# nucypher/TFHE.jl

Hardware: AMD Instinct MI355X
Metric: bootstrapped gates/sec (whole node), N=1024 (higher is better)
Workload: dtype int32 torus / f64 transform; 1 GPU; batch of 4096 independent gate_nand() bootstraps per GPU, tfhe_parameters_80 (n=500, N=1024, k=1, l=2, Bg=2^10, ks t=8, base 2^2); inputs=resident in HBM, launch=one process

## Files before the change

### tfhe.jl_amd/csrc/br_core.hpp

```cpp
#pragma once
#include <stdint.h>
#include <string.h>

#if defined(__HIPCC__)
#include <hip/hip_runtime.h>
#define TFHE_HD __host__ __device__ __forceinline__
typedef double2 cplx;
#else
#define TFHE_HD inline
struct cplx { double x, y; };
#endif

namespace tfhe {

constexpr int kWave = 64;
constexpr int kN = 1024;
constexpr int kM = kN / 2;
constexpr int kPts = kM / kWave;
constexpr int kXchElems = 576;

TFHE_HD cplx mk(double re, double im) { cplx c; c.x = re; c.y = im; return c; }
TFHE_HD cplx cadd(cplx a, cplx b) { return mk(a.x + b.x, a.y + b.y); }
TFHE_HD cplx csub(cplx a, cplx b) { return mk(a.x - b.x, a.y - b.y); }
TFHE_HD cplx cmul(cplx a, cplx b) { return mk(a.x * b.x - a.y * b.y, a.x * b.y + a.y * b.x); }
// ... 312 lines not shown
        const uint32_t v = (uint32_t)p[(B & (NBLK - 1)) * 64];
#if defined(__HIP_DEVICE_COMPILE__)
        uint32_t c_s = (uint32_t)offset - sgn;
        asm("" : "+s"(c_s));
        const uint32_t k = c_s - (uint32_t)cur[m];
        uint32_t r;
        asm("v_xad_u32 %0, %1, %2, %3" : "=v"(r) : "v"(v), "s"(sgn), "v"(k));
        temp[m] = (int32_t)(r ^ (uint32_t)xormask);
#else
        const uint32_t k = ((uint32_t)offset - sgn) - (uint32_t)cur[m];
        temp[m] = (int32_t)(((v ^ sgn) + k) ^ (uint32_t)xormask);
#endif
    }
}
template <int NBLK>
TFHE_HD void load_cur(int lane, const int32_t *img, int32_t (&cur)[NBLK])
{
#pragma unroll
    for (int m = 0; m < NBLK; m++) cur[m] = img[kMir + lane + 64 * m];
}
template <int NBLK>
TFHE_HD void store_cur(int lane, const int32_t (&acc)[NBLK], int32_t *img)
{
#pragma unroll
    for (int m = 0; m < NBLK; m++) img[kMir + lane + 64 * m] = acc[m];
    img[lane] = (int32_t)(0u - (uint32_t)acc[NBLK - 1]);
}

TFHE_HD int32_t digit2(int32_t t, int p, int log2_base)
{
#if defined(__HIP_DEVICE_COMPILE__)
    return __builtin_amdgcn_sbfe(t, (unsigned)(32 - p * log2_base), (unsigned)log2_base);
#else
    return (int32_t)((uint32_t)t << ((p - 1) * log2_base)) >> (32 - log2_base);
#endif
}
TFHE_HD void load_digits2(const int32_t (&temp)[16], int p, int log2_base, cplx (&x)[8])
{
#pragma unroll
    for (int r = 0; r < 8; r++) {
        const double lo = (double)digit2(temp[r], p, log2_base);
        const double hi = (double)digit2(temp[r + 8], p, log2_base);
        if (r == 0) x[r] = mk(lo, -hi);
        else x[r] = mk(lo * twc(r) - hi * tws(r), -(lo * tws(r) + hi * twc(r)));
    }
}
template <int R>
TFHE_HD cplx twist_tan(double a, double b)
{
    if (R == 0) return mk(a, -b);
    if (R == 4) return mk(a - b, -(b + a));
    if (R < 4) return mk(fma_(-twt(R), b, a), -fma_(twt(R), a, b));
    return mk(fma_(twt(R), a, -b), -fma_(twt(R), b, a));
}
TFHE_HD void load_digits2t(const int32_t (&temp)[16], int p, int log2_base, cplx (&u)[8])
{
#define TFHE_TW_(R) u[R] = twist_tan<R>((double)digit2(temp[R], p, log2_base), (double)digit2(temp[R + 8], p, log2_base))
    TFHE_TW_(0); TFHE_TW_(1); TFHE_TW_(2); TFHE_TW_(3); TFHE_TW_(4); TFHE_TW_(5); TFHE_TW_(6); TFHE_TW_(7);
#undef TFHE_TW_
}
constexpr double kTwR0 = 0.70710678118654752440;
constexpr double kTwR1 = 0.84775906502257351226;
constexpr double kTwR3 = 1.1795804271032745923;
constexpr double kTwG0 = 0.92387953251128675613;
constexpr double kTwL = 0.98078528040323044913;
constexpr double kTwSL = 0.69351992266107373091;
TFHE_HD cplx axpy(cplx a, double m, cplx b) { return mk(fma_(m, b.x, a.x), fma_(m, b.y, a.y)); }
TFHE_HD void dft8_fwd_tw(cplx (&x)[8])
{
    const cplx a0 = axpy(x[0], kTwR0, x[4]), a1 = axpy(x[1], kTwR1, x[5]), a2 = cadd(x[2], x[6]), a3 = axpy(x[3], kTwR3, x[7]);
    const cplx t0 = axpy(x[0], -kTwR0, x[4]), t1 = axpy(x[1], -kTwR1, x[5]), t2 = csub(x[2], x[6]), t3 = axpy(x[3], -kTwR3, x[7]);
    const cplx b1 = mk(t1.x + t1.y, t1.y - t1.x);
    const cplx b2 = mk(t2.y, -t2.x);
    const cplx b3 = mk(t3.y - t3.x, -(t3.x + t3.y));
    {
        const cplx c0 = axpy(a0, kTwG0, a2), d0 = axpy(a0, -kTwG0, a2), c1 = axpy(a1, kTwR1, a3), e = axpy(a1, -kTwR1, a3);
        const cplx d1 = mk(e.y, -e.x);
        x[0] = axpy(c0, kTwL, c1); x[4] = axpy(c0, -kTwL, c1); x[2] = axpy(d0, kTwL, d1); x[6] = axpy(d0, -kTwL, d1);
    }
    {
        const cplx c0 = axpy(t0, kTwG0, b2), d0 = axpy(t0, -kTwG0, b2), c1 = axpy(b1, kTwR1, b3), e = axpy(b1, -kTwR1, b3);
        const cplx d1 = mk(e.y, -e.x);
        x[1] = axpy(c0, kTwSL, c1); x[5] = axpy(c0, -kTwSL, c1); x[3] = axpy(d0, kTwSL, d1); x[7] = axpy(d0, -kTwSL, d1);
    }
}
TFHE_HD void fwd2_pass_a(cplx (&x)[8], const LaneTw &w)
{
    dft8<false>(x);
#pragma unroll
    for (int q = 0; q < 8; q++) x[q] = cmul(x[q], w.tw1f[q]);
}
TFHE_HD void fwd2_pass_b(cplx (&x)[8], const LaneTw &w)
{
    dft8<false>(x);
#pragma unroll
    for (int q = 1; q < 8; q++) x[q] = cmul(x[q], w.tw2[q]);
}
TFHE_HD void inv2_pass_b(cplx (&x)[8], const LaneTw &w)
{
#pragma unroll
    for (int q = 1; q < 8; q++) x[q] = cmulc(x[q], w.tw2[q]);
    dft8<true>(x);
}
TFHE_HD void inv2_pass_a(cplx (&x)[8], const LaneTw &w)
{
#pragma unroll
    for (int q = 0; q < 8; q++) x[q] = cmulc(x[q], w.tw1f[q]);
    dft8<true>(x);
}
TFHE_HD double frac_dist(double v)
{
    const double r = (v + 6755399441055744.0) - 6755399441055744.0;
    const double d = v - r;
    return d < 0 ? -d : d;
}

template <bool MARGIN = false, bool FUSED = true>
TFHE_HD void untwist_add2(const cplx (&y)[8], int32_t (&acc)[16], double *worst = nullptr)
{
#pragma unroll
    for (int r = 0; r < 8; r++) {
        if (FUSED) {
            double zr, zi;
            if (r == 0) { zr = y[r].x; zi = y[r].y; }
            else if (r == 4) { zr = y[r].x - y[r].y; zi = y[r].y + y[r].x; }
            else if (r < 4) { zr = fma_(-twt(r), y[r].y, y[r].x); zi = fma_(twt(r), y[r].x, y[r].y); }
            else { zr = fma_(twt(r), y[r].x, -y[r].y); zi = fma_(twt(r), y[r].y, y[r].x); }
            if (MARGIN) {
                const double a = frac_dist(zr * twk(r)), b = frac_dist(zi * twk(r));
                if (a > *worst) *worst = a;
                if (b > *worst) *worst = b;
            }
            acc[r] = (int32_t)((uint32_t)acc[r] + (uint32_t)round_scaled_to_torus32(zr, twk(r)));
            acc[r + 8] = (int32_t)((uint32_t)acc[r + 8] + (uint32_t)round_scaled_to_torus32(zi, -twk(r)));
        } else {
            double re, im;
            if (r == 0) { re = y[r].x; im = -y[r].y; }
            else { re = y[r].x * twc(r) - y[r].y * tws(r); im = -(y[r].x * tws(r) + y[r].y * twc(r)); }
            if (MARGIN) {
                const double a = frac_dist(re), b = frac_dist(im);
                if (a > *worst) *worst = a;
                if (b > *worst) *worst = b;
            }
            acc[r] = (int32_t)((uint32_t)acc[r] + (uint32_t)round_to_torus32(re));
            acc[r + 8] = (int32_t)((uint32_t)acc[r + 8] + (uint32_t)round_to_torus32(im));
        }
    }
}

}
```

### tfhe.jl_amd/csrc/engine.hpp

```cpp
#pragma once
#include <hip/hip_runtime.h>

#include <algorithm>
#include <atomic>
#include <cstdarg>
#include <cstdio>
#include <cstring>
#include <new>
#include <string>
#include <thread>
#include <vector>

#include "../../include/tfhe_mi355x.h"
#include "experiment.hpp"
#include "br_core.hpp"

using namespace tfhe;

#include "kernels_blind_rotate.hpp"
#include "kernels_anyn.hpp"
#include "kernels_n512.hpp"
#include "kernels_keyswitch.hpp"

struct ErrBuf {
// ... 149 lines not shown
    int n512_rw = 0;
    int k2_w3 = -1;
    int k2_rw = 0;
    int v3_rw = 0;
    int64_t pipeline_min = 4096;
    bool last_call_two_streams = false;
    struct MapStage { void *h = nullptr; size_t cap = 0; hipEvent_t ev = nullptr; bool pending = false; };
    static constexpr int kMapStages = 4;
    MapStage map_stage[kMapStages];
    unsigned map_next = 0;
    MapStage *map_cur = &map_stage[0];
    void *h_map = nullptr;
    hipEvent_t map_ev = nullptr;

    std::atomic<std::thread::id> owner{};
    int owner_depth = 0;

    bool multi() const { return !kids.empty(); }

    int set_err(int code, const char *fmt, ...)
    {
        ErrBuf next;
        va_list ap;
        va_start(ap, fmt);
        vsnprintf(next.s, sizeof next.s, fmt, ap);
        va_end(ap);
        err = next;
        return code;
    }
};

#define HIP_TRY(ctx, call)                                                                         \
    do {                                                                                           \
        hipError_t e_ = (call);                                                                    \
        if (e_ != hipSuccess)                                                                      \
            return (ctx)->set_err(TFHE_ERR_DEVICE, "%s failed: %s (%s:%d)", #call, hipGetErrorString(e_), __FILE__, __LINE__); \
    } while (0)


extern thread_local const tfhe_ctx *g_rejected_ctx;
extern const char kBusyMessage[];
struct CallGuard {
    tfhe_ctx *c;
    bool ok;
    explicit CallGuard(tfhe_ctx *c_) : c(c_), ok(false)
    {
        const std::thread::id me = std::this_thread::get_id();
        if (c->owner.load(std::memory_order_acquire) == me) { c->owner_depth++; ok = true; return; }
        std::thread::id none{};
        ok = c->owner.compare_exchange_strong(none, me, std::memory_order_acq_rel);
        if (ok) { c->owner_depth = 1; if (g_rejected_ctx == c) g_rejected_ctx = nullptr; }
        else g_rejected_ctx = c;
    }
    ~CallGuard()
    {
        if (ok && --c->owner_depth == 0) c->owner.store(std::thread::id{}, std::memory_order_release);
    }
    CallGuard(const CallGuard &) = delete;
    CallGuard &operator=(const CallGuard &) = delete;
};
#define ENTER_CTX(ctx)                                                                             \
    if (!(ctx)) return TFHE_ERR_INVALID_ARG;                                                       \
    alloc_checkpoint();                                                                            \
    CallGuard call_guard_(ctx);                                                                    \
    if (!call_guard_.ok) return TFHE_ERR_STATE

int32_t abi_caught(tfhe_ctx *c, const char *who) noexcept;
#define ABI_CATCH(ctx, who) catch (...) { return abi_caught(ctx, who); }
extern std::atomic<int64_t> g_fail_alloc_countdown;
inline void alloc_checkpoint()
{
    if (g_fail_alloc_countdown.load(std::memory_order_relaxed) > 0 && g_fail_alloc_countdown.fetch_sub(1, std::memory_order_relaxed) == 1) throw std::bad_alloc();
}

int32_t ensure_dyn_lds(tfhe_ctx *c, const void *fn, size_t bytes, const char *what);
#define LDS_TRY(ctx, bytes, ...)                                                                   \
    do {                                                                                           \
        const int32_t rl_ = ensure_dyn_lds(ctx, (const void *)(__VA_ARGS__), (size_t)(bytes), #__VA_ARGS__); \
        if (rl_) return rl_;                                                                       \
    } while (0)

constexpr size_t kH2TableOffset = kTableElems + 1024;
constexpr size_t kN512TableOffset = kH2TableOffset + kH2TableElems;

inline int ilog2i(int x) { int r = 0; while ((1 << r) < x) r++; return r; }
inline bool op_has_a(int op) { return !(op == TFHE_GATE_CONST0 || op == TFHE_GATE_CONST1); }
inline bool op_has_b(int op) { return op_has_a(op) && !(op == TFHE_GATE_NOT || op == TFHE_GATE_COPY); }
inline size_t bk_poly_count(const tfhe_params &p) { return (size_t)p.n * p.bs_l * (p.k + 1) * (p.k + 1); }

template <typename F>
struct ScopeExit {
    F f;
    ~ScopeExit() { f(); }
};
template <typename F>
ScopeExit<F> on_exit(F f) { return ScopeExit<F>{f}; }

template <typename F>
static int32_t fan_out(tfhe_ctx *c, const std::vector<int> &which, F &&fn)
{
    std::vector<int32_t> rcs(which.size(), TFHE_OK);
    std::vector<std::thread> th;
    std::vector<size_t> inline_ones;
    th.reserve(which.size());
    inline_ones.reserve(which.size());
    auto shard = [&](size_t i) noexcept {
        try { rcs[i] = fn(which[i]); } catch (...) { rcs[i] = abi_caught(c->kids[(size_t)which[i]], "fan-out shard"); }
    };
    for (size_t i = 1; i < which.size(); i++) {
        try {
            th.emplace_back([&shard, i] { shard(i); });
        } catch (...) {
            inline_ones.push_back(i);
        }
    }
    if (!which.empty()) shard(0);
    for (size_t i : inline_ones) shard(i);
    for (auto &t : th) t.join();
    std::fill(c->kid_ran.begin(), c->kid_ran.end(), 0);
    for (int k : which) c->kid_ran[(size_t)k] = 1;
    for (size_t i = 0; i < which.size(); i++)
        if (rcs[i]) return c->set_err(rcs[i], "device %d (kid %d): %s", c->kids[(size_t)which[i]]->device, which[i], c->kids[(size_t)which[i]]->err.c_str());
    return TFHE_OK;
}
inline std::vector<int> all_kids(const tfhe_ctx *c)
{
    std::vector<int> v(c->kids.size());
    for (size_t i = 0; i < v.size(); i++) v[i] = (int)i;
    return v;
}

template <typename F>
static int32_t multi_rows(tfhe_ctx *c, int64_t B, F &&call)
{
    const int nk = (int)c->kids.size();
    std::vector<int> which;
    std::vector<int64_t> lo((size_t)nk), hi((size_t)nk);
    for (int r = 0; r < nk; r++) {
        lo[(size_t)r] = B * r / nk; hi[(size_t)r] = B * (r + 1) / nk;
        if (hi[(size_t)r] > lo[(size_t)r]) which.push_back(r);
    }
    return fan_out(c, which, [&](int r) { return call(c->kids[(size_t)r], lo[(size_t)r], hi[(size_t)r] - lo[(size_t)r]); });
}

void shard_bounds_by_rotations(const uint8_t *opcodes, int64_t B, int shards, int64_t *bounds);
void quiesce(tfhe_ctx *c);
int32_t tgsw_prepare(tfhe_ctx *c, const int32_t *d_polys, cplx *d_out, size_t npolys, hipStream_t s);
void mk_tgsw_drop(tfhe_ctx *c);
struct DiagArgs;
int32_t prepare_diag(tfhe_ctx *c, size_t R, hipStream_t s, DiagArgs &d);
void name_kernel(tfhe_ctx *c, const char *fmt, ...) __attribute__((format(printf, 2, 3)));
struct TvPtrs { const int32_t *tv; const int32_t *index; int32_t *bodies = nullptr; int32_t n_out = 1; };
template <class A>
static WithTv<A> with_tv(const A &a, const TvPtrs &tv)
{
    WithTv<A> t;
    static_cast<A &>(t) = a;
    t.tv = tv.tv;
    t.tv_index = tv.index;
    t.bodies = tv.bodies;
    t.n_out = tv.n_out;
    return t;
}
int32_t launch_blind_rotate(tfhe_ctx *c, size_t R, int32_t mu, hipStream_t s, const TvPtrs *tv = nullptr);
int32_t launch_keyswitch(tfhe_ctx *c, size_t G, const int32_t *e0, const int32_t *e1, const int32_t *dst, const int32_t *ext, int32_t *out, hipStream_t s);
int32_t enter_stream(tfhe_ctx *c, hipStream_t s);
// ... 45 lines not shown
```

### tfhe.jl_amd/csrc/engine_context.hip

```cpp
#include "engine.hpp"
#include <cmath>

thread_local ErrBuf g_create_error;
thread_local const tfhe_ctx *g_rejected_ctx = nullptr;
static thread_local const tfhe_ctx *g_caught_ctx = nullptr;
static thread_local ErrBuf g_caught_error;
std::atomic<int64_t> g_fail_alloc_countdown{0};
const char kBusyMessage[] = "the context is inside another call on another thread: calls on one context must not overlap (one caller at a time; use one context per thread)";

int32_t abi_caught(tfhe_ctx *c, const char *who) noexcept
{
    int32_t code = TFHE_ERR_STATE;
    ErrBuf &e = c ? g_caught_error : g_create_error;
    try {
        throw;
    } catch (const std::bad_alloc &) {
        code = TFHE_ERR_NOMEM;
        e.format("%s: out of host memory (std::bad_alloc); nothing was changed that a repeated call would not redo", who);
    } catch (const std::exception &x) {
        e.format("%s: unexpected C++ exception: %s", who, x.what());
    } catch (...) {
        e.format("%s: unexpected C++ exception", who);
    }
    g_caught_ctx = c;
    if (c) {
        const tfhe_ctx *rejected = g_rejected_ctx;
        CallGuard again(c);
        if (again.ok) c->err = g_caught_error;
        g_rejected_ctx = rejected;
    }
    return code;
}

static void build_tables(std::vector<cplx> &h)
{
    h.resize(kN512TableOffset + kN512TableElems);
    fill_tables<long double>(h.data(), [](long double a) { return cosl(a); }, [](long double a) { return sinl(a); });
    const long double pi = 3.14159265358979323846264338327950288L;
    for (int w = 0; w < 2; w++)
        for (int q = 0; q < 8; q++)
            for (int t = 0; t < 64; t++) {
                const long double a = -pi * (long double)(t * (1 + 4 * w + 8 * q)) / 2048.0L;
                h[kTableElems + w * 512 + q * 64 + t] = mk((double)cosl(a), (double)sinl(a));
            }
    auto put = [&](size_t idx, long double turns_of_pi) { const long double a = -pi * turns_of_pi; h[idx] = mk((double)cosl(a), (double)sinl(a)); };
    for (int hh = 0; hh < 2; hh++)
        for (int q = 0; q < 4; q++)
            for (int t = 0; t < 64; t++)
                put(kH2TableOffset + (size_t)(hh * 4 + q) * 64 + t, (long double)t / 1024.0L + (hh ? (long double)t / 256.0L : 0.0L) + (long double)(t * q) / 128.0L);
    for (int q = 0; q < 4; q++)
        for (int t = 0; t < 16; t++) put(kH2TableOffset + 512 + (size_t)q * 16 + t, (long double)(t * q) / 32.0L);
    for (int q = 0; q < 4; q++)
        for (int t = 0; t < 4; t++) put(kH2TableOffset + 576 + (size_t)q * 4 + t, (long double)(t * q) / 8.0L);
    for (int q = 0; q < 4; q++)
        for (int t = 0; t < 64; t++) put(kN512TableOffset + (size_t)q * 64 + t, (long double)t / 512.0L + (long double)(t * q) / 128.0L);
}

void shard_bounds_by_rotations(const uint8_t *opcodes, int64_t B, int shards, int64_t *bounds)
{
    auto cost = [&](int64_t g) -> int64_t {
        const int op = opcodes ? opcodes[g] : TFHE_GATE_NAND;
        const int rot = op == TFHE_GATE_MUX ? 2 : (op == TFHE_GATE_NOT || op == TFHE_GATE_COPY || op == TFHE_GATE_CONST0 || op == TFHE_GATE_CONST1) ? 0 : 1;
        return 1000 * (int64_t)rot + 1;
    };
    int64_t total = 0;
    for (int64_t g = 0; g < B; g++) total += cost(g);
    bounds[0] = 0;
    int64_t cum = 0, g = 0;
    for (int r = 1; r < shards; r++) {
        while (g < B && cum * shards < total * r) { cum += cost(g); g++; }
        bounds[r] = g;
    }
    bounds[shards] = B;
}

extern "C" {

int32_t tfhe_abi_version(void) { return TFHE_ABI_VERSION_REPORTED; }

int32_t tfhe_device_count(void)
{
    int n = 0;
    if (hipGetDeviceCount(&n) != hipSuccess) return -1;
    return n;
}

const char *tfhe_last_error(const tfhe_ctx *ctx)
{
    if (!ctx) return g_create_error.c_str();
    if (g_rejected_ctx == ctx) return kBusyMessage;
    if (g_caught_ctx == ctx) return g_caught_error.c_str();
    return ctx->err.c_str();
}

int32_t tfhe_shard_bounds(const uint8_t *opcodes, int64_t B, int32_t shards, int64_t *bounds) try
{
    alloc_checkpoint();
    if (B < 0 || shards < 1 || !bounds) return TFHE_ERR_INVALID_ARG;
    shard_bounds_by_rotations(opcodes, B, shards, bounds);
    return TFHE_OK;
}
ABI_CATCH(nullptr, "tfhe_shard_bounds")

static void exactness_class(const tfhe_params &p, int &cls, double &bound_log2, double &margin)
{
    const double np = (double)(p.parties > 1 ? p.parties + 1 : p.k + 1) * p.bs_l, N = (double)p.N, beta = (double)p.bs_log2_base;
    bound_log2 = std::log2(np * N) + (beta - 1.0) + 31.0;
    const double rms = std::sqrt(np * N) * std::exp2(beta + 32.0) / 12.0;
    margin = 4.5 * std::exp2(-53.0) * rms * std::max(4.0, std::log2(N / 2.0));
    const bool margin_ok = margin < 0.25, typical_ok = 8.0 * rms < std::exp2(51.0);
    cls = !(margin_ok && typical_ok) ? 0 : bound_log2 < 51.0 ? 2 : 1;
}

int32_t tfhe_ctx_create(const tfhe_params *params, int32_t device_id, tfhe_ctx **out_ctx) try
{
    alloc_checkpoint();
    if (!params || !out_ctx) { g_create_error = "tfhe_ctx_create: NULL argument"; return TFHE_ERR_INVALID_ARG; }
    *out_ctx = nullptr;
    const tfhe_params &p = *params;
    char buf[256];
// ... 217 lines not shown
```

### tfhe.jl_amd/csrc/engine_dispatch.hip

```cpp
#define TFHE_EMIT_KEYSWITCH_KERNELS
#include "engine.hpp"
#include "br_launch.hpp"

#include <map>
#include <mutex>
#include <functional>

int32_t ensure_dyn_lds(tfhe_ctx *c, const void *fn, size_t bytes, const char *what)
{
    static std::mutex mu;
    static std::map<std::pair<int, const void *>, size_t> have;
    std::lock_guard<std::mutex> lk(mu);
    size_t &cur = have[std::make_pair(c->device, fn)];
    if (cur >= bytes) return TFHE_OK;
    const hipError_t e = hipFuncSetAttribute(fn, hipFuncAttributeMaxDynamicSharedMemorySize, (int)bytes);
    if (e != hipSuccess) return c->set_err(TFHE_ERR_DEVICE, "hipFuncSetAttribute(%s, %zu bytes of LDS) failed: %s", what, bytes, hipGetErrorString(e));
    cur = bytes;
    return TFHE_OK;
}

int32_t prepare_diag(tfhe_ctx *c, size_t R, hipStream_t s, DiagArgs &d)
{
    d.margin_bits = nullptr; d.clk = nullptr; d.phase = nullptr;
    c->diag_rows = 0;
    if (!c->measure_margin) return TFHE_OK;
    HIP_TRY(c, c->diag.reserve(R * 24 + 64 * 8));
    HIP_TRY(c, hipMemsetAsync(c->diag.p, 0, R * 24 + 64 * 8, s));
    d.margin_bits = (unsigned long long *)c->diag.p;
    d.clk = d.margin_bits + R;
    d.phase = d.clk + 2 * R;
    c->diag_rows = R;
    return TFHE_OK;
}

void name_kernel(tfhe_ctx *c, const char *fmt, ...)
{
    char buf[128];
    va_list ap;
    va_start(ap, fmt);
    vsnprintf(buf, sizeof buf, fmt, ap);
    va_end(ap);
    c->last_kernel = buf;
}

static int br_inst_l(const tfhe_ctx *c)
{
    return (c->P.bs_l == 2 || c->P.bs_l == 3) && !c->br_rt_l ? c->P.bs_l : 0;
}

static void name_br(tfhe_ctx *c, const char *family, int L, const char *rest = "")
{
    if (L) name_kernel(c, "blind_rotate_kernel_%s<%d%s>", family, L, rest);
    else name_kernel(c, "blind_rotate_kernel_%s<0%s>(l=%d)", family, rest, c->P.bs_l);
}

static int32_t launch_blind_rotate_part(tfhe_ctx *c, size_t first, size_t R, int32_t mu, hipStream_t s, const DiagArgs &diag, int k2_kind = -1 ,
                                        const TvPtrs *tv_all = nullptr)
{
    TvPtrs tv{nullptr, nullptr};
    if (tv_all) tv = TvPtrs{tv_all->tv, tv_all->index + first, tv_all->bodies ? tv_all->bodies + first * (size_t)tv_all->n_out : nullptr, tv_all->n_out};
    BrArgs a;
    a.diag = diag;
    if (diag.margin_bits) { a.diag.margin_bits += first; a.diag.clk += 2 * first; }
    const bool dg = c->measure_margin;
    a.bara = (const int32_t *)c->bara.p + first * (size_t)(c->P.n + 1);
    a.bk = c->d_bk;
    a.ext = (int32_t *)c->ext.p + first * ((size_t)c->P.k * c->P.N + 1);
    a.T = c->T;
    a.g = c->g;
    a.n = c->P.n;
    a.mu = mu;
    a.prio_steps = (int32_t)((int64_t)c->P.n * c->br_prio_pct / 100);
    a.R = (int32_t)R;
    const int L = c->P.bs_l;
    a.l = L;
    if (c->anyn()) {
        const int K1 = c->P.k + 1, N = c->P.N, M = N / 2;
        anyn::Args g;
        g.diag = a.diag; g.bara = a.bara; g.bk = a.bk; g.ext = a.ext; g.g = c->g; g.n = a.n; g.mu = mu; g.K1 = K1; g.L = L; g.R = (int32_t)R;
        g.log2N = ilog2i(N); g.parties = 1;
        g.wtab = c->d_anyn_tab; g.twist = c->d_anyn_tab + M;
        HIP_TRY(c, c->mk_acc.reserve((first + R) * (size_t)K1 * N * sizeof(int32_t)));
        g.acc = (int32_t *)c->mk_acc.p + first * (size_t)K1 * N;
        const bool fits = anyn::lds_bytes(N, K1) <= 160 * 1024;
        const bool spec_lds = c->anyn_spec < 0 ? fits : (c->anyn_spec == 0 && fits);
        g.spec_g = nullptr;
        if (!spec_lds) {
            HIP_TRY(c, c->spec.reserve((first + R) * (size_t)K1 * (M > 0 ? M : 1) * sizeof(cplx)));
            g.spec_g = (cplx *)c->spec.p + first * (size_t)K1 * (M > 0 ? M : 1);
        }
        const BrLaunch geo{0, 1, dg, dim3((unsigned)R), dim3((unsigned)anyn::threads_for(N)), anyn::lds_bytes(N, spec_lds ? K1 : 0)};
        const int32_t rc = tv_all ? br_launch_anyn(c, with_tv(g, tv), geo, s) : br_launch_anyn(c, g, geo, s);
        if (rc) return rc;
        name_kernel(c, spec_lds ? "blind_rotate_kernel_anyn(N=%d,k=%d,l=%d)" : "blind_rotate_kernel_anyn(N=%d,k=%d,l=%d,spec=global)", N, c->P.k, L);
        return TFHE_OK;
    }
    if (c->n512()) {
        N512Args b;
        b.diag = a.diag; b.bara = a.bara; b.bk = a.bk; b.ext = a.ext; b.g = c->g; b.n = a.n; b.mu = mu; b.R = (int32_t)R; b.l = L;
        b.prio_steps = a.prio_steps;
        b.tw1 = c->d_tables + kN512TableOffset; b.tw2q = c->d_tables + kH2TableOffset + 512; b.tw3q = b.tw2q + 64;
        if (c->n512_w2 == 1 || (c->n512_w2 < 0 && R <= 6 * (size_t)c->cu_count)) {
            const BrLaunch geo{br_inst_l(c), 1, dg, dim3((unsigned)R), dim3(128), kN512W2LdsBytes};
            const int32_t rc = tv_all ? br_launch_n512w2(c, with_tv(b, tv), geo, s) : br_launch_n512w2(c, b, geo, s);
            if (rc) return rc;
            name_br(c, "n512w2", geo.L);
            return TFHE_OK;
        }
        const bool group = !dg && (c->n512_rw == 4 || (c->n512_rw == 0 && R >= 8 * (size_t)c->cu_count));
        const int rw = group ? 4 : 1;
        const BrLaunch geo{br_inst_l(c), rw, dg, dim3((unsigned)((R + rw - 1) / rw)), dim3(64 * rw), (size_t)rw * kN512LdsBytes};
        const int32_t rc = tv_all ? br_launch_n512(c, with_tv(b, tv), geo, s) : br_launch_n512(c, b, geo, s);
        if (rc) return rc;
        name_br(c, "n512", geo.L, group ? ",rw4" : "");
        return TFHE_OK;
    }
    const bool tuned = c->P.N == kN2 ? (c->P.k == 1 && L == 3) : c->P.k == 1 ? true : (c->P.k == 2 && (L == 2 || L == 3));
    if (!tuned || c->br_general) {
        const int K1 = c->P.k + 1, H = c->P.N / kN;
        const size_t img = (size_t)kMir + c->P.N;
        BrGenArgs g;
        g.diag = a.diag; g.bara = a.bara; g.bk = a.bk; g.ext = a.ext; g.g = c->g; g.n = a.n; g.mu = mu; g.K1 = K1; g.L = L; g.R = (int32_t)R;
        HIP_TRY(c, c->mk_acc.reserve((first + R) * K1 * img * sizeof(int32_t)));
        g.acc = (int32_t *)c->mk_acc.p + first * K1 * img;
        g.tw1f = c->P.N == kN2 ? (const cplx *)(c->d_tables + kTableElems) : c->T.tw1f;
        g.tw2 = c->T.tw2;
        const BrLaunch geo{0, 1, dg, dim3((unsigned)R), dim3(64), (kXchElems + 64 + (size_t)K1 * H * kM) * sizeof(cplx)};
        const bool n2048 = c->P.N == kN2;
        const int32_t rc = tv_all ? br_launch_general(c, with_tv(g, tv), n2048, geo, s) : br_launch_general(c, g, n2048, geo, s);
        if (rc) return rc;
        name_kernel(c, "blind_rotate_kernel_general(N=%d,k=%d,l=%d)", c->P.N, c->P.k, L);
        return TFHE_OK;
    }
    if (c->P.N == kN2) {
        Br2048Args b;
        b.diag = a.diag; b.bara = a.bara; b.bk = a.bk; b.ext = a.ext; b.tw1f2 = c->d_tables + kTableElems; b.tw2 = c->T.tw2; b.g = c->g; b.n = a.n; b.mu = mu; b.prio_steps = a.prio_steps;
        b.R = (int32_t)R;
        const int rw = dg ? 1 : c->n2048_rw ? c->n2048_rw : (R <= (size_t)c->cu_count ? 1 : 2);
        const size_t ldsb = (size_t)rw * (2 * kImg2 * 4 + 2 * kXchElems * sizeof(cplx)) + 64 * sizeof(cplx) + 64;
        const BrLaunch geo{L, rw, dg, dim3((unsigned)((R + rw - 1) / rw)), dim3(128 * rw), ldsb};
        const int32_t rc = tv_all ? br_launch_n2048x(c, with_tv(b, tv), geo, s) : br_launch_n2048x(c, b, geo, s);
        if (rc) return rc;
        name_br(c, "n2048x", L, rw == 2 ? ",rw2" : ",rw1");
        return TFHE_OK;
    }
    if (c->P.k == 2) {
        const size_t cus = (size_t)c->cu_count;
        const bool w3 = k2_kind >= 0 ? k2_kind == 1 : (c->k2_w3 == 1 || (c->k2_w3 < 0 && R <= 2 * cus));
        if (w3) {
            const BrLaunch geo{L, 1, dg, dim3((unsigned)R), dim3(192), kK2W3LdsBytes};
            const int32_t rc = tv_all ? br_launch_k2w3(c, with_tv(a, tv), geo, s) : br_launch_k2w3(c, a, geo, s);
// ... 177 lines not shown
```

### tfhe.jl_amd/csrc/kernels_common.hpp

```cpp
#pragma once

#include <hip/hip_runtime.h>

#include "../../include/tfhe_mi355x.h"
#include <type_traits>

#include "br_core.hpp"

using namespace tfhe;

template <class A>
struct WithTv : A {
    const int32_t *tv;
    const int32_t *tv_index;
    int32_t *bodies;
    int32_t n_out;
};
#ifdef TFHE_TV_KERNELS
#define TV_KERNEL(name) name##_tv
#define TV_ARGS(A) WithTv<A>
constexpr bool kTV = true;
#else
#define TV_KERNEL(name) name
#define TV_ARGS(A) A
constexpr bool kTV = false;
#endif
template <class A>
__device__ __forceinline__ const int32_t *tv_of(const A &, size_t, int) { return nullptr; }
template <class A>
__device__ __forceinline__ const int32_t *tv_of(const WithTv<A> &P, size_t w, int N)
{
    return P.tv + (size_t)__builtin_amdgcn_readfirstlane(P.tv_index[w]) * N;
}
template <class A>
__device__ __forceinline__ void store_bodies(const A &, size_t, int, const int32_t *, int) {}
template <class A>
__device__ __forceinline__ void store_bodies(const WithTv<A> &P, size_t w, int lane, const int32_t *body, int N)
{
    if (P.bodies && lane < P.n_out) P.bodies[w * P.n_out + lane] = body[lane * (N / P.n_out)];
}

struct DiagArgs {
    unsigned long long *margin_bits;
    unsigned long long *clk;
    unsigned long long *phase;
};

#ifdef TFHE_STAMP
#define STAMP_DECL unsigned long long st_prev_ = __builtin_amdgcn_s_memtime(), st_acc_[16] = {0, 0, 0, 0, 0, 0, 0, 0, 0, 0, 0, 0, 0, 0, 0, 0}
#define STAMP(k) do { if (MARGIN) { const unsigned long long t_ = __builtin_amdgcn_s_memtime(); st_acc_[k] += t_ - st_prev_; st_prev_ = t_; } } while (0)
#define STAMP_FLUSH(diag, wave) do { if (MARGIN && blockIdx.x == 0 && (threadIdx.x & 63) == 0 && (diag).phase) { for (int k_ = 0; k_ < 16; k_++) (diag).phase[(wave) * 16 + k_] = st_acc_[k_]; } } while (0)
#else
#define STAMP_DECL do { } while (0)
#define STAMP(k) do { } while (0)
#define STAMP_FLUSH(diag, wave) do { } while (0)
#endif

template <bool DIAG>
__device__ __forceinline__ void diag_begin(unsigned long long &t0, unsigned long long &r0)
{
    if constexpr (DIAG) {
        t0 = __builtin_amdgcn_s_memtime();
        r0 = __builtin_amdgcn_s_memrealtime();
    }
}
template <bool DIAG>
__device__ __forceinline__ void diag_end(const DiagArgs &d, size_t w, double worst, unsigned long long t0, unsigned long long r0, bool clock_writer = (threadIdx.x == 0))
{
    if constexpr (DIAG) {
#pragma unroll
        for (int off = 32; off > 0; off >>= 1) {
            const double o = __shfl_xor(worst, off);
            worst = o > worst ? o : worst;
        }
        if ((threadIdx.x & 63) == 0) {
            atomicMax(&d.margin_bits[w], (unsigned long long)__double_as_longlong(worst));
            if (clock_writer) {
                d.clk[2 * w] = __builtin_amdgcn_s_memtime() - t0;
                d.clk[2 * w + 1] = __builtin_amdgcn_s_memrealtime() - r0;
            }
        }
    }
}

__device__ __forceinline__ int wave_in_block() { return __builtin_amdgcn_readfirstlane((int)(threadIdx.x >> 6)); }
__device__ __forceinline__ int32_t load_uniform_i32(const int32_t *p)
{
    return *(const __attribute__((address_space(4))) int32_t *)(p);
}

__device__ __forceinline__ int lane_id() { return (int)__builtin_amdgcn_mbcnt_hi(~0u, __builtin_amdgcn_mbcnt_lo(~0u, 0u)); }
__device__ __forceinline__ int lane_id_fresh()
{
    unsigned z = 0;
    asm volatile("" : "+s"(z));
    return (int)__builtin_amdgcn_mbcnt_hi(~0u, __builtin_amdgcn_mbcnt_lo(~0u, z));
}

template <int I, int N, typename F>
__device__ __forceinline__ void static_for(F &&f)
{
    if constexpr (I < N) {
        f(std::integral_constant<int, I>{});
        static_for<I + 1, N>(f);
    }
}

__device__ __forceinline__ double opaque_scalar(double v) { asm("" : "+s"(v)); return v; }
struct Tan16 { double t[5], r0, r1, r3, g0, l, sl, c[5]; };
template <bool WITH_COS = false>
__device__ __forceinline__ Tan16 load_tan16()
{
    Tan16 k;
    k.t[0] = 0.0; k.t[4] = 1.0; k.c[0] = 1.0;
    if (WITH_COS) { k.c[1] = opaque_scalar(twk(1)); k.c[2] = opaque_scalar(twk(2)); k.c[3] = opaque_scalar(twk(3)); k.c[4] = opaque_scalar(twk(4)); }
    k.t[1] = opaque_scalar(twt(1)); k.t[2] = opaque_scalar(twt(2)); k.t[3] = opaque_scalar(twt(3));
    k.r0 = opaque_scalar(kTwR0); k.r1 = opaque_scalar(kTwR1); k.r3 = opaque_scalar(kTwR3);
    k.g0 = opaque_scalar(kTwG0); k.l = opaque_scalar(kTwL); k.sl = opaque_scalar(kTwSL);
    return k;
}
template <int R>
__device__ __forceinline__ cplx twist_tan_o(double a, double b, const Tan16 &k)
{
    if (R == 0) return mk(a, -b);
    if (R == 4) return mk(a - b, -(b + a));
    const double t = k.t[R < 4 ? R : 8 - R];
    if (R < 4) return mk(fma_(-t, b, a), -fma_(t, a, b));
    return mk(fma_(t, a, -b), -fma_(t, b, a));
}
__device__ __forceinline__ void load_digits2t_o(const int32_t (&temp)[16], int p, int log2_base, cplx (&u)[8], const Tan16 &k)
{
    static_for<0, 8>([&](auto rc) {
        constexpr int R = decltype(rc)::value;
        u[R] = twist_tan_o<R>((double)digit2(temp[R], p, log2_base), (double)digit2(temp[R + 8], p, log2_base), k);
    });
}
__device__ __forceinline__ void dft8_fwd_tw_o(cplx (&x)[8], const Tan16 &k)
{
    const cplx a0 = axpy(x[0], k.r0, x[4]), a1 = axpy(x[1], k.r1, x[5]), a2 = cadd(x[2], x[6]), a3 = axpy(x[3], k.r3, x[7]);
    const cplx t0 = axpy(x[0], -k.r0, x[4]), t1 = axpy(x[1], -k.r1, x[5]), t2 = csub(x[2], x[6]), t3 = axpy(x[3], -k.r3, x[7]);
    const cplx b1 = mk(t1.x + t1.y, t1.y - t1.x);
    const cplx b2 = mk(t2.y, -t2.x);
    const cplx b3 = mk(t3.y - t3.x, -(t3.x + t3.y));
    {
        const cplx c0 = axpy(a0, k.g0, a2), d0 = axpy(a0, -k.g0, a2), c1 = axpy(a1, k.r1, a3), e = axpy(a1, -k.r1, a3);
        const cplx d1 = mk(e.y, -e.x);
        x[0] = axpy(c0, k.l, c1); x[4] = axpy(c0, -k.l, c1); x[2] = axpy(d0, k.l, d1); x[6] = axpy(d0, -k.l, d1);
    }
    {
        const cplx c0 = axpy(t0, k.g0, b2), d0 = axpy(t0, -k.g0, b2), c1 = axpy(b1, k.r1, b3), e = axpy(b1, -k.r1, b3);
        const cplx d1 = mk(e.y, -e.x);
        x[1] = axpy(c0, k.sl, c1); x[5] = axpy(c0, -k.sl, c1); x[3] = axpy(d0, k.sl, d1); x[7] = axpy(d0, -k.sl, d1);
    }
}

template <bool MARGIN>
__device__ __forceinline__ void untwist_add2_o(const cplx (&y)[8], int32_t (&acc)[16], double *worst, const Tan16 &k)
{
    static_for<0, 8>([&](auto rc) {
        constexpr int r = decltype(rc)::value;
        const double t = k.t[r < 4 ? r : 8 - r], c = k.c[r < 4 ? r : 8 - r];
        double zr, zi;
        if (r == 0) { zr = y[r].x; zi = y[r].y; }
        else if (r == 4) { zr = y[r].x - y[r].y; zi = y[r].y + y[r].x; }
        else if (r < 4) { zr = fma_(-t, y[r].y, y[r].x); zi = fma_(t, y[r].x, y[r].y); }
        else { zr = fma_(t, y[r].x, -y[r].y); zi = fma_(t, y[r].y, y[r].x); }
        if (MARGIN) {
            const double a = frac_dist(zr * c), b = frac_dist(zi * c);
            if (a > *worst) *worst = a;
            if (b > *worst) *worst = b;
        }
        if (r == 0) {
            acc[r] = (int32_t)((uint32_t)acc[r] + (uint32_t)round_to_torus32(zr));
            acc[r + 8] = (int32_t)((uint32_t)acc[r + 8] + (uint32_t)round_to_torus32(-zi));
        } else {
            acc[r] = (int32_t)((uint32_t)acc[r] + (uint32_t)round_scaled_to_torus32(zr, c));
            acc[r + 8] = (int32_t)((uint32_t)acc[r + 8] + (uint32_t)round_scaled_to_torus32(zi, -c));
        }
    });
}

struct BrArgs {
    DiagArgs diag;
    const int32_t *bara;
    const cplx *bk;
    int32_t *ext;
    Tables T;
    Gadget g;
    int32_t n;
    int32_t mu;
    int32_t prio_steps;
    int32_t R;
    int32_t l;
    int32_t grp_big, grp_q;
};

__device__ __forceinline__ void wave_priority_begin(int prio_steps)
{
    if (prio_steps > 0) __builtin_amdgcn_s_setprio(3);
}
__device__ __forceinline__ void wave_priority_step(int step, int prio_steps)
{
    if (prio_steps <= 0) return;
    if (step == prio_steps / 3) __builtin_amdgcn_s_setprio(2);
    else if (step == 2 * prio_steps / 3) __builtin_amdgcn_s_setprio(1);
    else if (step == prio_steps) __builtin_amdgcn_s_setprio(0);
}

#define WAVE_LDS_FENCE() asm volatile("" ::: "memory")

constexpr int kImg = kMir + kN;

template <int NBLK>
__device__ __forceinline__ void rotate_poly(int lane, int a, const int32_t *img, int32_t offset, int32_t xormask, int32_t (&temp)[NBLK])
{
    int32_t cur[NBLK];
    load_cur<NBLK>(lane, img, cur);
    int a_here = __builtin_amdgcn_readfirstlane(a);
    asm volatile("" : "+s"(a_here));
    rotate_sub3<NBLK>(lane, a_here, img, cur, offset, xormask, temp);
}
template <bool MARGIN, bool FUSED = true>
__device__ __forceinline__ void accumulate_poly(int lane, const cplx (&y)[8], int32_t *img, double *worst)
{
    int32_t accr[16];
    load_cur<16>(lane, img, accr);
    untwist_add2<MARGIN, FUSED>(y, accr, worst);
    store_cur<16>(lane, accr, img);
}
__device__ __forceinline__ void init_body_poly(int lane, int barb, int32_t mu, int32_t *img)
{
    int32_t b[16];
#pragma unroll
    for (int m = 0; m < 16; m++) {
        const int idx = (lane + 64 * m + barb) & (2 * kN - 1);
        b[m] = (idx & kN) ? (int32_t)(0u - (uint32_t)mu) : mu;
    }
    store_cur<16>(lane, b, img);
}
__device__ __forceinline__ int32_t tv_coef(const int32_t *v, int idx, int N)
{
    const int32_t x = v[idx & (N - 1)];
    return (idx & N) ? (int32_t)(0u - (uint32_t)x) : x;
}
template <class A>
__device__ __forceinline__ void init_body(int lane, int barb, const A &P, size_t w, int32_t *img)
{
    if constexpr (kTV) {
        const int32_t *v = tv_of(P, w, kN);
        int32_t b[16];
#pragma unroll
        for (int m = 0; m < 16; m++) b[m] = tv_coef(v, (lane + 64 * m + barb) & (2 * kN - 1), kN);
        store_cur<16>(lane, b, img);
    } else {
        init_body_poly(lane, barb, P.mu, img);
    }
}
__device__ __forceinline__ void init_zero_poly(int lane, int32_t *img)
{
    int32_t z[16];
#pragma unroll
    for (int m = 0; m < 16; m++) z[m] = 0;
    store_cur<16>(lane, z, img);
}
__device__ __forceinline__ void extract_mask_poly(int lane, const int32_t *img, int32_t *ext)
{
#pragma unroll
    for (int m = 0; m < 16; m++) {
        const int j = lane + 64 * m;
        const int32_t v = img[kMir + j];
// ... 95 lines not shown
```

### tfhe.jl_amd/csrc/kernels_v3.hpp

```cpp
#pragma once
#include "kernels_common.hpp"

constexpr int kV3SyncEvery = 4;
constexpr int kV3LdsBytes = 2 * kImg * 4 + (kXchElems + 64) * (int)sizeof(cplx);

template <int L, int KPF , bool TW2REG = false ,
          bool MARGIN = false , int RW = 1 >
__global__ __launch_bounds__(64 * RW, 2) void TV_KERNEL(blind_rotate_kernel_v3)(TV_ARGS(BrArgs) P)
{
    constexpr int K1 = 2;
    constexpr int KMID = (KPF == 8) ? 4 : 0;
    const int Lr = L ? L : P.l;
    const int F = K1 * Lr;
    wave_priority_begin(P.prio_steps);
    unsigned long long dg_t0 = 0, dg_r0 = 0;
    diag_begin<MARGIN>(dg_t0, dg_r0);
    extern __shared__ __attribute__((aligned(16))) char smem_all[];
        const int wib = (RW > 1) ? wave_in_block() : 0;
    char *smem = smem_all + (size_t)wib * kV3LdsBytes;
    int32_t *acc_lds = reinterpret_cast<int32_t *>(smem);
    cplx *xch = reinterpret_cast<cplx *>(smem + K1 * kImg * 4);
    cplx *tw2_lds = xch + kXchElems;
    const int lane = (RW > 1) ? lane_id() : (int)threadIdx.x;
    size_t w = (size_t)blockIdx.x * RW + wib;
    const bool padding = (RW > 1) && w >= (size_t)P.R;
    if (padding) w = P.R - 1;
    const int32_t *bara = P.bara + w * (P.n + 1);
    const int beta = P.g.log2_base;
    const int32_t xormask = gadget_xor_mask(Lr, beta);

    cplx tw1f[8];
#pragma unroll
    for (int q = 0; q < 8; q++) tw1f[q] = P.T.tw1f[q * 64 + lane];
    tw2_lds[lane] = P.T.tw2[lane];
    cplx tw2r[8];
    if (TW2REG) {
#pragma unroll
        for (int q = 1; q < 8; q++) tw2r[q] = P.T.tw2[q * 8 + (lane & 7)];
    }
    init_zero_poly(lane, acc_lds);
    init_body(lane, bara[P.n] & (2 * kN - 1), P, w, acc_lds + kImg);
    WAVE_LDS_FENCE();

    double worst = 0.0;
    cplx kbuf[16];
    auto key_ptr = [&](int step, int f) {
        const int c = L ? f / (L ? L : 1) : (f >= Lr), p = L ? f % (L ? L : 1) : f - c * Lr;
        return P.bk + (size_t)step * (Lr * K1 * K1 * kM) + (size_t)(p * K1 + c) * K1 * kM + lane;
    };
    {
        const cplx *kp = key_ptr(0, 0);
#pragma unroll
        for (int j = 0; j < KPF; j++) kbuf[j] = kp[j * 64];
    }

    int a_next = bara[0] & (2 * kN - 1);
    for (int i = 0; i < P.n; i++) {
        const int a = a_next;
        a_next = bara[i + 1] & (2 * kN - 1);
        wave_priority_step(i, P.prio_steps);
        if (RW > 1 && (i % kV3SyncEvery) == 0) __builtin_amdgcn_s_barrier();

        cplx out[K1][8];
        int32_t temp[16];
#pragma unroll 1
        for (int f = 0; f < F; f++) {
            const int c = L ? f / (L ? L : 1) : (f >= Lr), p = L ? f % (L ? L : 1) : f - c * Lr;
            if (p == 0) rotate_poly<16>(lane, a, acc_lds + c * kImg, P.g.offset, xormask, temp);
            cplx x[8];
            load_digits2t(temp, p + 1, beta, x);
            dft8_fwd_tw(x);
#pragma unroll
            for (int q = 0; q < 8; q++) x[q] = cmul(x[q], tw1f[q]);
            x1_store_a(lane, x, xch);
            WAVE_LDS_FENCE();
            x1_load_b(lane, x, xch);
            {
                cplx t2[8];
#pragma unroll
                for (int q = 1; q < 8; q++) t2[q] = TW2REG ? tw2r[q] : tw2_lds[q * 8 + (lane & 7)];
                dft8<false>(x);
#pragma unroll
                for (int q = 1; q < 8; q++) x[q] = cmul(x[q], t2[q]);
            }
            WAVE_LDS_FENCE();
            x2_store(lane, x, xch);
            WAVE_LDS_FENCE();
            cplx k1v[8];
            if (KPF == 8 && KMID > 0) {
                const cplx *kp = key_ptr(i, f);
#pragma unroll
                for (int k2 = 0; k2 < KMID; k2++) k1v[k2] = kp[(8 + k2) * 64];
                WAVE_LDS_FENCE();
            }
            x2_load(lane, x, xch);
            WAVE_LDS_FENCE();
            dft8<false>(x);
            if (KPF == 16) {
                if (f == 0) {
#pragma unroll
                    for (int co = 0; co < K1; co++)
#pragma unroll
                        for (int k2 = 0; k2 < 8; k2++) out[co][k2] = cmul(x[k2], kbuf[co * 8 + k2]);
                } else {
#pragma unroll
                    for (int co = 0; co < K1; co++)
#pragma unroll
                        for (int k2 = 0; k2 < 8; k2++) out[co][k2] = cfma(x[k2], kbuf[co * 8 + k2], out[co][k2]);
                }
            } else {
                const cplx *kp = key_ptr(i, f);
#pragma unroll
                for (int k2 = KMID; k2 < 8; k2++) k1v[k2] = kp[(8 + k2) * 64];
                if (f == 0) {
#pragma unroll
                    for (int k2 = 0; k2 < 8; k2++) out[0][k2] = cmul(x[k2], kbuf[k2]);
#pragma unroll
                    for (int k2 = 0; k2 < 8; k2++) out[1][k2] = cmul(x[k2], k1v[k2]);
                } else {
#pragma unroll
                    for (int k2 = 0; k2 < 8; k2++) out[0][k2] = cfma(x[k2], kbuf[k2], out[0][k2]);
#pragma unroll
                    for (int k2 = 0; k2 < 8; k2++) out[1][k2] = cfma(x[k2], k1v[k2], out[1][k2]);
                }
            }
            {
                const bool last = (f + 1 == F);
                const cplx *kp = last ? key_ptr(i + 1 < P.n ? i + 1 : i, 0) : key_ptr(i, f + 1);
#pragma unroll
                for (int j = 0; j < KPF; j++) kbuf[j] = kp[j * 64];
            }
        }
#pragma unroll
        for (int co = 0; co < K1; co++) {
            dft8<true>(out[co]);
            x2_store(lane, out[co], xch);
            WAVE_LDS_FENCE();
            x2_load(lane, out[co], xch);
            {
                cplx t2[8];
#pragma unroll
                for (int q = 1; q < 8; q++) t2[q] = TW2REG ? tw2r[q] : tw2_lds[q * 8 + (lane & 7)];
#pragma unroll
                for (int q = 1; q < 8; q++) out[co][q] = cmulc(out[co][q], t2[q]);
            }
            dft8<true>(out[co]);
            WAVE_LDS_FENCE();
            x1_store_b(lane, out[co], xch);
            WAVE_LDS_FENCE();
            x1_load_a(lane, out[co], xch);
            WAVE_LDS_FENCE();
#pragma unroll
            for (int q = 0; q < 8; q++) out[co][q] = cmulc(out[co][q], tw1f[q]);
            dft8<true>(out[co]);
            accumulate_poly<MARGIN>(lane, out[co], acc_lds + co * kImg, &worst);
        }
        WAVE_LDS_FENCE();
    }

    if (padding) return;
    int32_t *ext = P.ext + w * (kN + 1);
    extract_mask_poly(lane, acc_lds, ext);
    if (lane == 0) ext[kN] = acc_lds[kImg + kMir];
    store_bodies(P, w, lane, acc_lds + kImg + kMir, kN);
    diag_end<MARGIN>(P.diag, w, worst, dg_t0, dg_r0);
}
```

Before: 366,500 gates/s.

## Fold radix-8 twiddles into tangent-scaled DFT8 for middle FFT pass

Replaces the separate second-stage twiddle complex multiply plus plain DFT8 with a per-lane tangent-based scaling (one FMA pair per point) followed by a DFT8 whose butterflies absorb the cosine ratios. This applies in both the forward and inverse middle passes and removes the twiddle LDS reads and cmuls. It also moves the margin tracking into LDS to free registers. The cost is a new precomputed table and possible precision changes from the tangent/ratio factorisation.

Measured after the change: 371,900 gates/s (median of 6 runs). +1.5%, better.

```diff
diff --git a/tfhe.jl_amd/csrc/br_core.hpp b/tfhe.jl_amd/csrc/br_core.hpp
--- a/tfhe.jl_amd/csrc/br_core.hpp
+++ b/tfhe.jl_amd/csrc/br_core.hpp
@@ -418,6 +418,80 @@
         const cplx c0 = axpy(t0, kTwG0, b2), d0 = axpy(t0, -kTwG0, b2), c1 = axpy(b1, kTwR1, b3), e = axpy(b1, -kTwR1, b3);
         const cplx d1 = mk(e.y, -e.x);
         x[1] = axpy(c0, kTwSL, c1); x[5] = axpy(c0, -kTwSL, c1); x[3] = axpy(d0, kTwSL, d1); x[7] = axpy(d0, -kTwSL, d1);
+    }
+}
+constexpr int kTan2Doubles = 16;
+constexpr int kTan2Elems = 8 * kTan2Doubles / 2;
+struct LaneTan2 {
+    double t[6];
+    double r1, r2, r3;
+    double g0, g1, l, sl;
+    cplx w4;
+};
+template <typename LD, typename COS, typename SIN>
+inline void fill_tan2(double *h, COS cosfn, SIN sinfn)
+{
+    const LD pi = (LD)3.14159265358979323846264338327950288L;
+    for (int s = 0; s < 8; s++) {
+        LD c[8], t[8];
+        for (int v = 0; v < 8; v++) {
+            const LD a = (LD)2 * pi * (LD)(v * s) / (LD)64;
+            c[v] = cosfn(a); t[v] = sinfn(a) / cosfn(a);
+        }
+        double *o = h + s * kTan2Doubles;
+        const LD a4 = (LD)-2 * pi * (LD)(4 * s) / (LD)64;
+        o[14] = (double)cosfn(a4); o[15] = (double)sinfn(a4);
+        c[0] = 1; c[4] = 1;
+        o[0] = (double)t[1]; o[1] = (double)t[2]; o[2] = (double)t[3]; o[3] = (double)t[5]; o[4] = (double)t[6]; o[5] = (double)t[7];
+        for (int v = 0; v < 4; v++) o[6 + v] = (double)(c[v + 4] / c[v]);
+        o[10] = (double)(c[2] / c[0]); o[11] = (double)(c[3] / c[1]);
+        o[12] = (double)(c[1] / c[0]); o[13] = (double)(c[1] / c[0] * (LD)0.70710678118654752440084436210484904L);
+    }
+}
+TFHE_HD void load_lane_tan2(int lane, const double *tab, LaneTan2 &k)
+{
+    const double *o = tab + (lane & 7) * kTan2Doubles;
+#pragma unroll
+    for (int j = 0; j < 6; j++) k.t[j] = o[j];
+    k.r1 = o[7]; k.r2 = o[8]; k.r3 = o[9]; k.g0 = o[10]; k.g1 = o[11]; k.l = o[12]; k.sl = o[13];
+    k.w4 = mk(o[14], o[15]);
+}
+template <bool INV>
+TFHE_HD cplx tan2_point(cplx x, double t)
+{
+    return INV ? mk(fma_(-t, x.y, x.x), fma_(t, x.x, x.y)) : mk(fma_(t, x.y, x.x), fma_(-t, x.x, x.y));
+}
+template <bool INV>
+TFHE_HD void tan2_apply(cplx (&x)[8], const LaneTan2 &k)
+{
+    x[1] = tan2_point<INV>(x[1], k.t[0]); x[2] = tan2_point<INV>(x[2], k.t[1]); x[3] = tan2_point<INV>(x[3], k.t[2]);
+    x[4] = INV ? cmulc(x[4], k.w4) : cmul(x[4], k.w4);
+    x[5] = tan2_point<INV>(x[5], k.t[3]); x[6] = tan2_point<INV>(x[6], k.t[4]); x[7] = tan2_point<INV>(x[7], k.t[5]);
+}
+template <bool INV>
+TFHE_HD void dft8_scaled(cplx (&x)[8], const LaneTan2 &k)
+{
+    const cplx a0 = cadd(x[0], x[4]), a1 = axpy(x[1], k.r1, x[5]), a2 = axpy(x[2], k.r2, x[6]), a3 = axpy(x[3], k.r3, x[7]);
+    const cplx t0 = csub(x[0], x[4]), t1 = axpy(x[1], -k.r1, x[5]), t2 = axpy(x[2], -k.r2, x[6]), t3 = axpy(x[3], -k.r3, x[7]);
+    cplx b1, b2, b3;
+    if (!INV) {
+        b1 = mk(t1.x + t1.y, t1.y - t1.x);
+        b2 = mk(t2.y, -t2.x);
+        b3 = mk(t3.y - t3.x, -(t3.x + t3.y));
+    } else {
+        b1 = mk(t1.x - t1.y, t1.x + t1.y);
+        b2 = mk(-t2.y, t2.x);
+        b3 = mk(-(t3.x + t3.y), t3.x - t3.y);
+    }
+    {
+        const cplx c0 = axpy(a0, k.g0, a2), d0 = axpy(a0, -k.g0, a2), c1 = axpy(a1, k.g1, a3), e = axpy(a1, -k.g1, a3);
+        const cplx d1 = INV ? mk(-e.y, e.x) : mk(e.y, -e.x);
+        x[0] = axpy(c0, k.l, c1); x[4] = axpy(c0, -k.l, c1); x[2] = axpy(d0, k.l, d1); x[6] = axpy(d0, -k.l, d1);
+    }
+    {
+        const cplx c0 = axpy(t0, k.g0, b2), d0 = axpy(t0, -k.g0, b2), c1 = axpy(b1, k.g1, b3), e = axpy(b1, -k.g1, b3);
+        const cplx d1 = INV ? mk(-e.y, e.x) : mk(e.y, -e.x);
+        x[1] = axpy(c0, k.sl, c1); x[5] = axpy(c0, -k.sl, c1); x[3] = axpy(d0, k.sl, d1); x[7] = axpy(d0, -k.sl, d1);
     }
 }
 TFHE_HD void fwd2_pass_a(cplx (&x)[8], const LaneTw &w)
diff --git a/tfhe.jl_amd/csrc/engine.hpp b/tfhe.jl_amd/csrc/engine.hpp
--- a/tfhe.jl_amd/csrc/engine.hpp
+++ b/tfhe.jl_amd/csrc/engine.hpp
@@ -255,6 +255,7 @@
 
 constexpr size_t kH2TableOffset = kTableElems + 1024;
 constexpr size_t kN512TableOffset = kH2TableOffset + kH2TableElems;
+constexpr size_t kTan2TableOffset = kN512TableOffset + kN512TableElems;
 
 inline int ilog2i(int x) { int r = 0; while ((1 << r) < x) r++; return r; }
 inline bool op_has_a(int op) { return !(op == TFHE_GATE_CONST0 || op == TFHE_GATE_CONST1); }
diff --git a/tfhe.jl_amd/csrc/engine_context.hip b/tfhe.jl_amd/csrc/engine_context.hip
--- a/tfhe.jl_amd/csrc/engine_context.hip
+++ b/tfhe.jl_amd/csrc/engine_context.hip
@@ -34,8 +34,9 @@
 
 static void build_tables(std::vector<cplx> &h)
 {
-    h.resize(kN512TableOffset + kN512TableElems);
+    h.resize(kTan2TableOffset + kTan2Elems);
     fill_tables<long double>(h.data(), [](long double a) { return cosl(a); }, [](long double a) { return sinl(a); });
+    fill_tan2<long double>(reinterpret_cast<double *>(h.data() + kTan2TableOffset), [](long double a) { return cosl(a); }, [](long double a) { return sinl(a); });
     const long double pi = 3.14159265358979323846264338327950288L;
     for (int w = 0; w < 2; w++)
         for (int q = 0; q < 8; q++)
diff --git a/tfhe.jl_amd/csrc/engine_dispatch.hip b/tfhe.jl_amd/csrc/engine_dispatch.hip
--- a/tfhe.jl_amd/csrc/engine_dispatch.hip
+++ b/tfhe.jl_amd/csrc/engine_dispatch.hip
@@ -67,6 +67,7 @@
     a.bk = c->d_bk;
     a.ext = (int32_t *)c->ext.p + first * ((size_t)c->P.k * c->P.N + 1);
     a.T = c->T;
+    a.tan2 = reinterpret_cast<const double *>(c->d_tables + kTan2TableOffset);
     a.g = c->g;
     a.n = c->P.n;
     a.mu = mu;
diff --git a/tfhe.jl_amd/csrc/kernels_common.hpp b/tfhe.jl_amd/csrc/kernels_common.hpp
--- a/tfhe.jl_amd/csrc/kernels_common.hpp
+++ b/tfhe.jl_amd/csrc/kernels_common.hpp
@@ -65,7 +65,8 @@
     }
 }
 template <bool DIAG>
-__device__ __forceinline__ void diag_end(const DiagArgs &d, size_t w, double worst, unsigned long long t0, unsigned long long r0, bool clock_writer = (threadIdx.x == 0))
+__device__ __forceinline__ void diag_end(const DiagArgs &d, size_t w, double worst, unsigned long long t0, unsigned long long r0, bool clock_writer = (threadIdx.x == 0),
+                                         int lane_in_wave = (int)(threadIdx.x & 63))
 {
     if constexpr (DIAG) {
 #pragma unroll
@@ -73,7 +74,7 @@
             const double o = __shfl_xor(worst, off);
             worst = o > worst ? o : worst;
         }
-        if ((threadIdx.x & 63) == 0) {
+        if (lane_in_wave == 0) {
             atomicMax(&d.margin_bits[w], (unsigned long long)__double_as_longlong(worst));
             if (clock_writer) {
                 d.clk[2 * w] = __builtin_amdgcn_s_memtime() - t0;
@@ -186,6 +187,7 @@
     const cplx *bk;
     int32_t *ext;
     Tables T;
+    const double *tan2;
     Gadget g;
     int32_t n;
     int32_t mu;
diff --git a/tfhe.jl_amd/csrc/kernels_v3.hpp b/tfhe.jl_amd/csrc/kernels_v3.hpp
--- a/tfhe.jl_amd/csrc/kernels_v3.hpp
+++ b/tfhe.jl_amd/csrc/kernels_v3.hpp
@@ -4,7 +4,7 @@
 constexpr int kV3SyncEvery = 4;
 constexpr int kV3LdsBytes = 2 * kImg * 4 + (kXchElems + 64) * (int)sizeof(cplx);
 
-template <int L, int KPF , bool TW2REG = false ,
+template <int L, int KPF , bool TW2REG = true ,
           bool MARGIN = false , int RW = 1 >
 __global__ __launch_bounds__(64 * RW, 2) void TV_KERNEL(blind_rotate_kernel_v3)(TV_ARGS(BrArgs) P)
 {
@@ -20,7 +20,6 @@
     char *smem = smem_all + (size_t)wib * kV3LdsBytes;
     int32_t *acc_lds = reinterpret_cast<int32_t *>(smem);
     cplx *xch = reinterpret_cast<cplx *>(smem + K1 * kImg * 4);
-    cplx *tw2_lds = xch + kXchElems;
     const int lane = (RW > 1) ? lane_id() : (int)threadIdx.x;
     size_t w = (size_t)blockIdx.x * RW + wib;
     const bool padding = (RW > 1) && w >= (size_t)P.R;
@@ -32,17 +31,14 @@
     cplx tw1f[8];
 #pragma unroll
     for (int q = 0; q < 8; q++) tw1f[q] = P.T.tw1f[q * 64 + lane];
-    tw2_lds[lane] = P.T.tw2[lane];
-    cplx tw2r[8];
-    if (TW2REG) {
-#pragma unroll
-        for (int q = 1; q < 8; q++) tw2r[q] = P.T.tw2[q * 8 + (lane & 7)];
-    }
+    LaneTan2 tk;
+    load_lane_tan2(lane, P.tan2, tk);
+    double *worst_lds = reinterpret_cast<double *>(xch + kXchElems);
+    if (MARGIN) worst_lds[lane] = 0.0;
     init_zero_poly(lane, acc_lds);
     init_body(lane, bara[P.n] & (2 * kN - 1), P, w, acc_lds + kImg);
     WAVE_LDS_FENCE();
 
-    double worst = 0.0;
     cplx kbuf[16];
     auto key_ptr = [&](int step, int f) {
         const int c = L ? f / (L ? L : 1) : (f >= Lr), p = L ? f % (L ? L : 1) : f - c * Lr;
@@ -75,14 +71,7 @@
             x1_store_a(lane, x, xch);
             WAVE_LDS_FENCE();
             x1_load_b(lane, x, xch);
-            {
-                cplx t2[8];
-#pragma unroll
-                for (int q = 1; q < 8; q++) t2[q] = TW2REG ? tw2r[q] : tw2_lds[q * 8 + (lane & 7)];
-                dft8<false>(x);
-#pragma unroll
-                for (int q = 1; q < 8; q++) x[q] = cmul(x[q], t2[q]);
-            }
+            dft8<false>(x);
             WAVE_LDS_FENCE();
             x2_store(lane, x, xch);
             WAVE_LDS_FENCE();
@@ -95,7 +84,9 @@
             }
             x2_load(lane, x, xch);
             WAVE_LDS_FENCE();
-            dft8<false>(x);
+            __builtin_amdgcn_sched_barrier(0);
+            tan2_apply<false>(x, tk);
+            dft8_scaled<false>(x, tk);
             if (KPF == 16) {
                 if (f == 0) {
 #pragma unroll
@@ -137,14 +128,8 @@
             x2_store(lane, out[co], xch);
             WAVE_LDS_FENCE();
             x2_load(lane, out[co], xch);
-            {
-                cplx t2[8];
-#pragma unroll
-                for (int q = 1; q < 8; q++) t2[q] = TW2REG ? tw2r[q] : tw2_lds[q * 8 + (lane & 7)];
-#pragma unroll
-                for (int q = 1; q < 8; q++) out[co][q] = cmulc(out[co][q], t2[q]);
-            }
-            dft8<true>(out[co]);
+            tan2_apply<true>(out[co], tk);
+            dft8_scaled<true>(out[co], tk);
             WAVE_LDS_FENCE();
             x1_store_b(lane, out[co], xch);
             WAVE_LDS_FENCE();
@@ -153,7 +138,9 @@
 #pragma unroll
             for (int q = 0; q < 8; q++) out[co][q] = cmulc(out[co][q], tw1f[q]);
             dft8<true>(out[co]);
+            double worst = MARGIN ? worst_lds[lane] : 0.0;
             accumulate_poly<MARGIN>(lane, out[co], acc_lds + co * kImg, &worst);
+            if (MARGIN) worst_lds[lane] = worst;
         }
         WAVE_LDS_FENCE();
     }
@@ -163,5 +150,6 @@
     extract_mask_poly(lane, acc_lds, ext);
     if (lane == 0) ext[kN] = acc_lds[kImg + kMir];
     store_bodies(P, w, lane, acc_lds + kImg + kMir, kN);
-    diag_end<MARGIN>(P.diag, w, worst, dg_t0, dg_r0);
+    if constexpr (RW > 1 && L != 0) diag_end<MARGIN>(P.diag, w, MARGIN ? worst_lds[lane] : 0.0, dg_t0, dg_r0, wib == 0 && lane == 0, lane);
+    else diag_end<MARGIN>(P.diag, w, MARGIN ? worst_lds[lane] : 0.0, dg_t0, dg_r0);
 }
```
